# TravisWheelerLab/BATH

Measured on AMD Instinct MI355X. Metric: DP Gcells/s + residues/s through bathsearch pipeline at 1/2/4/8 MI355X, higher is better.
Workload: dtype u8/i16 integer scores (SSV: exact binary16), f32 Forward

## Files before the change

bath_amd/csrc/bath_viterbi.hip:

```cpp
#include <algorithm>
#include <cstdlib>
#include <functional>

#include "bath_common.hpp"
#include "bath_kernels.hpp"
#include "bath_launch.hpp"

using namespace bath;

namespace bath {

__device__ __forceinline__ s16x2 pk_adds(s16x2 a, s16x2 b) { return __builtin_elementwise_add_sat(a, b); }
__device__ __forceinline__ s16x2 pk_max(s16x2 a, s16x2 b) { return __builtin_elementwise_max(a, b); }
__device__ __forceinline__ s16x2 as_s2(unsigned v) { return __builtin_bit_cast(s16x2, v); }
__device__ __forceinline__ unsigned as_u(s16x2 v) { return __builtin_bit_cast(unsigned, v); }

struct VitLaneTables {
  const int16_t *rw;
  int rw_pitch_bytes;
  const uint32_t *tw2;
  const int16_t *rank;
};

struct VitLaneConsts {
  int M, base_w, xwE_loop, xwE_move, Q8;
  float scale_w;
  double invP_vit, invP_msv;
  float scale_b;
  int base_b, tec_b, bias_b;
};

typedef uint32_t u32x16 __attribute__((ext_vector_type(16)));

template <int NR>
#ifndef BATH_VIT_WAVES
#define BATH_VIT_WAVES 1
#endif
__global__ __launch_bounds__(256, (NR <= 76 ? BATH_VIT_WAVES : 1)) void vit_lane_kernel(SeqView sq, VitLaneTables tb, const uint32_t *__restrict__ tw2g, VitLaneConsts c, const int16_t *__restrict__ xwmove_tab,
                                                          const uint8_t *__restrict__ tjb_tab, const int32_t *__restrict__ todo, int64_t ntodo,
                                                          const int *__restrict__ ntodo_dev, const int *__restrict__ skip_dev, float *__restrict__ sc, int32_t *__restrict__ status,
                                                          const float *__restrict__ filtersc, const uint8_t *__restrict__ ssv_scores,
                                                          WindowRec *__restrict__ wins, int *__restrict__ win_count, int win_cap, int32_t *__restrict__ kminmax) {
  extern __shared__ __attribute__((aligned(16))) char lds[];
  char *s_rw = lds;
  int16_t *s_rank = reinterpret_cast<int16_t *>(lds + 30 * tb.rw_pitch_bytes);
  {
    const uint32_t *src = reinterpret_cast<const uint32_t *>(tb.rw);
    uint32_t *dst = reinterpret_cast<uint32_t *>(s_rw);
    for (int i = threadIdx.x; i < 30 * tb.rw_pitch_bytes / 4; i += blockDim.x) dst[i] = src[i];
    for (int i = threadIdx.x; i < 2 * NR; i += blockDim.x) s_rank[i] = tb.rank[i];
  }
  __syncthreads();
  if (ntodo_dev) ntodo = *ntodo_dev;
  const int64_t t = (int64_t)blockIdx.x * blockDim.x + threadIdx.x + (skip_dev ? *skip_dev : 0);
  if (t - (threadIdx.x & 63) >= ntodo) return;
  const bool live = t < ntodo;
  const int64_t sid = live ? (todo ? (int64_t)todo[t] : t) : (todo ? (int64_t)todo[0] : 0);
  const int L = live ? sq.len[sid] : 0;
  const uint8_t *s = sq.data + sq.off[sid];
  const int Lw = wave_max_i32(L);
  const bool do_win = (wins != nullptr);
  const int M = c.M;

  const int xw_move = xwmove_tab[L];
  int sc_thresh = 0, sc_ext_thresh = 0, skip_until = 0, kmin = 1 << 30, kmax = 0;
  if (do_win && live) {
    const double fsc = (double)filtersc[sid];
    sc_thresh = (int)(int16_t)(int)ceil(((fsc + 0.69314718055994529 * c.invP_vit + 3.0) * (double)c.scale_w) -
                                        (double)(float)c.xwE_move - (double)(float)xw_move + (double)(float)c.base_w);
    sc_ext_thresh = (int)ceil(((fsc + 0.69314718055994529 * c.invP_msv + 3.0) * (double)c.scale_b) + c.base_b + c.tec_b + (int)tjb_tab[L]);
  }
  const s16x2 NEG = {-32768, -32768};
  s16x2 Mr[NR], Ir[NR], Dr[NR];
#pragma unroll
  for (int r = 0; r < NR; r++) Mr[r] = Ir[r] = Dr[r] = NEG;
  int xN = c.base_w;
  int xB = (int16_t)(xN + xw_move);
  int xJ = -32768, xC = -32768;
  bool overflow = false;
  short ePrev = -32768;

  uint32_t wnext = (0 < L) ? *reinterpret_cast<const uint32_t *>(s) : 0x1d1d1d1du;
  for (int i0 = 0; i0 < Lw; i0 += 4) {
    const uint32_t w = wnext;
    wnext = (i0 + 4 < L) ? *reinterpret_cast<const uint32_t *>(s + i0 + 4) : 0x1d1d1d1du;
#pragma unroll 1
    for (int j = 0; j < 4; j++) {
      const int i = i0 + j + 1;
      const bool on = (i <= L) && !overflow;
      int x = (w >> (8 * j)) & 0xff;
      x = (i <= L) ? min(x, kKp - 1) : 29;
      const char *rowbase = s_rw + x * tb.rw_pitch_bytes;
      const s16x2 xBv = {(short)xB, (short)xB};
      s16x2 xEv = NEG;
      unsigned pM = (as_u(Mr[NR - 1]) << 16) | 0x8000u, pI = (as_u(Ir[NR - 1]) << 16) | 0x8000u, pD = (as_u(Dr[NR - 1]) << 16) | 0x8000u;
      s16x2 dpk = NEG;
      s16x2 cpk = {(short)-32768, ePrev};
      int twz = 0;
      asm volatile("" : "+s"(twz));
      const uint32_t *tw = tw2g + twz;
      u32x16 t_c, t_n;
      int4 e_c = *reinterpret_cast<const int4 *>(rowbase), e_n = e_c;
      asm volatile("s_load_dwordx16 %0, %1, 0x0" : "=s"(t_c) : "s"(tw));
#pragma unroll
      for (int r = 0; r < NR; r += 2) {
        asm volatile("s_waitcnt lgkmcnt(0)" ::: "memory");
        __builtin_amdgcn_sched_barrier(0);
        if ((r & 3) == 0 && r + 4 < NR) e_n = *reinterpret_cast<const int4 *>(rowbase + 4 * (r + 4));
        if (r + 2 < NR) asm volatile("s_load_dwordx16 %0, %1, %2" : "=s"(t_n) : "s"(tw), "i"((r + 2) * 32));
        __builtin_amdgcn_sched_barrier(0);
        const unsigned em[2] = {(r & 3) ? (unsigned)e_c.z : (unsigned)e_c.x, (r & 3) ? (unsigned)e_c.w : (unsigned)e_c.y};
#pragma unroll
        for (int q = 0; q < 2; q++) {
          const int rr = r + q;
          const unsigned tMM = t_c[8 * q + 0], tIM = t_c[8 * q + 1], tDM = t_c[8 * q + 2], tBM = t_c[8 * q + 3];
          const unsigned tMD = t_c[8 * q + 4], tDD = t_c[8 * q + 5], tMI = t_c[8 * q + 6], tII = t_c[8 * q + 7];
          const unsigned oM = as_u(Mr[rr]), oI = as_u(Ir[rr]);
          const unsigned oD = as_u(pk_max(Dr[rr], cpk));
          cpk = pk_adds(cpk, as_s2(tDD));
          const s16x2 ms = as_s2(pM), is = as_s2(pI), ds = as_s2(pD);
          s16x2 sv = pk_adds(xBv, as_s2(tBM));
          sv = pk_max(sv, pk_adds(ms, as_s2(tMM)));
          sv = pk_max(sv, pk_adds(is, as_s2(tIM)));
          sv = pk_max(sv, pk_adds(ds, as_s2(tDM)));
          sv = pk_adds(sv, as_s2(em[q]));
          Ir[rr] = pk_max(pk_adds(as_s2(oM), as_s2(tMI)), pk_adds(as_s2(oI), as_s2(tII)));
          const s16x2 dcv = pk_adds(sv, as_s2(tMD));
          xEv = pk_max(xEv, sv);
          Mr[rr] = sv;
          Dr[rr] = dpk;
          dpk = pk_max(dcv, pk_adds(dpk, as_s2(tDD)));
          pM = oM; pI = oI; pD = oD;
        }
        if (r + 2 < NR) t_c = t_n;
        if ((r & 3) == 2 && r + 2 < NR) e_c = e_n;
        asm volatile("" : "+v"(Mr[r]), "+v"(Mr[r + 1]), "+v"(Ir[r]), "+v"(Ir[r + 1]), "+v"(Dr[r]), "+v"(Dr[r + 1]), "+v"(dpk), "+v"(cpk), "+v"(xEv));
        __builtin_amdgcn_sched_barrier(0);
      }
      ePrev = dpk.x;
      if (on) {
        const int xE = max((int)xEv.x, (int)xEv.y);
        if (xE >= 32767) overflow = true;
        else {
          xN = (int16_t)(xN + 0);
          xC = (int16_t)max(xC + 0, xE + c.xwE_move);
          xJ = (int16_t)max(xJ + 0, xE + c.xwE_loop);
          xB = (int16_t)max(xJ + xw_move, xN + xw_move);
          if (do_win && i > skip_until && xE >= sc_thresh) {
            int rank = 32767;
#pragma unroll
            for (int r = 0; r < NR; r++) {
              if ((int)Mr[r].x == xE) rank = min(rank, (int)s_rank[2 * r]);
              if ((int)Mr[r].y == xE) rank = min(rank, (int)s_rank[2 * r + 1]);
            }
            const int k_start = (rank / 8) + c.Q8 * (rank % 8) + 1;
            int max_k_end = k_start, max_i_end = i, sc_ext = sc_ext_thresh, max_sc_ext = sc_ext, since = 0;
            int kk = k_start + 1, nn = i + 1;
            while (kk <= M && nn <= L) {
              sc_ext += c.bias_b - (int)ssv_scores[(size_t)kk * kKp + min((int)s[nn - 1], kKp - 1)];
              if (sc_ext >= max_sc_ext) { max_sc_ext = sc_ext; max_k_end = kk; max_i_end = nn; since = 0; }
              else if (++since == 5) break;
              kk++; nn++;
            }
            const int slot = atomicAdd(win_count, 1);
            if (slot < win_cap) wins[slot] = WindowRec{(int32_t)sid, i, max_k_end, max_k_end - k_start + 1, 0.0f};
            kmax = max(kmax, max_k_end);
            kmin = min(kmin, k_start);
            skip_until = max_i_end;
          }
        }
      }
    }
  }
  if (live) {
    if (overflow) { sc[sid] = INFINITY; status[sid] = BATH_ERANGE; }
    else if (xC > -32768) {
      float r = (float)xC + (float)xw_move - (float)c.base_w;
      r /= c.scale_w;
      r = (float)((double)r - 3.0);
      sc[sid] = r; status[sid] = BATH_OK;
    } else { sc[sid] = -INFINITY; status[sid] = BATH_OK; }
    if (do_win && kminmax) { kminmax[2 * sid] = kmin; kminmax[2 * sid + 1] = kmax; }
  }
}

constexpr int kLenBins = 2048;
constexpr int kVitLongTarget = 128;
__device__ __forceinline__ void len_block_range(int n, int &lo, int &hi) {
  const int per = (n + (int)gridDim.x - 1) / (int)gridDim.x;
  lo = min(n, (int)blockIdx.x * per); hi = min(n, lo + per);
}
__global__ __launch_bounds__(256) void len_hist_kernel(const int32_t *__restrict__ todo, const int *__restrict__ ntodo_dev, const int32_t *__restrict__ len,
                                                       int *__restrict__ hist) {
  __shared__ int s_cnt[kLenBins];
  for (int i = threadIdx.x; i < kLenBins; i += blockDim.x) s_cnt[i] = 0;
  __syncthreads();
  int lo, hi;
  len_block_range(*ntodo_dev, lo, hi);
  for (int j = lo + threadIdx.x; j < hi; j += blockDim.x) atomicAdd(&s_cnt[min(len[todo[j]], kLenBins - 1)], 1);
  __syncthreads();
  for (int i = threadIdx.x; i < kLenBins; i += blockDim.x) if (s_cnt[i]) atomicAdd(&hist[i], s_cnt[i]);
}
__global__ void len_scan_kernel(int *__restrict__ hist ) {
  __shared__ int tmp[kLenBins];
  for (int i = threadIdx.x; i < kLenBins; i += blockDim.x) tmp[i] = hist[i];
  __syncthreads();
  if (threadIdx.x == 0) {
    int run = 0;
    for (int b = kLenBins - 1; b >= 0; b--) { const int cnt = tmp[b]; tmp[b] = run; run += cnt; }
  }
  __syncthreads();
  for (int i = threadIdx.x; i < kLenBins; i += blockDim.x) hist[i] = tmp[i];
}
__global__ __launch_bounds__(256) void len_scatter_kernel(const int32_t *__restrict__ todo, const int *__restrict__ ntodo_dev, const int32_t *__restrict__ len,
                                                          int *__restrict__ cursor, int32_t *__restrict__ sorted) {
  __shared__ int s_cnt[kLenBins];
  for (int i = threadIdx.x; i < kLenBins; i += blockDim.x) s_cnt[i] = 0;
  __syncthreads();
  int lo, hi;
  len_block_range(*ntodo_dev, lo, hi);
  for (int j = lo + threadIdx.x; j < hi; j += blockDim.x) atomicAdd(&s_cnt[min(len[todo[j]], kLenBins - 1)], 1);
  __syncthreads();
  for (int i = threadIdx.x; i < kLenBins; i += blockDim.x) { const int c = s_cnt[i]; if (c) s_cnt[i] = atomicAdd(&cursor[i], c); }
  __syncthreads();
  for (int j = lo + threadIdx.x; j < hi; j += blockDim.x) {
    const int cnd = todo[j];
    sorted[atomicAdd(&s_cnt[min(len[cnd], kLenBins - 1)], 1)] = cnd;
  }
}

int vit_lane_supported(const bath_hip_oprofile *om) { return om->vit_NR > 0; }

const int *len_sort_count_longer(const int *d_bins, int T) { return d_bins + std::min(T + 1, kLenBins - 1); }

int launch_len_sort(bath_hip_ctx *ctx, const int32_t *d_todo, const int *d_ntodo, const int32_t *d_len, int *d_bins, int32_t *d_sorted) {
  BATH_HIP_TRY(ctx, hipMemsetAsync(d_bins, 0, kLenBins * sizeof(int), ctx->stream));
  hipLaunchKernelGGL(len_hist_kernel, dim3(256), dim3(256), 0, ctx->stream, d_todo, d_ntodo, d_len, d_bins);
  hipLaunchKernelGGL(len_scan_kernel, dim3(1), dim3(256), 0, ctx->stream, d_bins);
  hipLaunchKernelGGL(len_scatter_kernel, dim3(256), dim3(256), 0, ctx->stream, d_todo, d_ntodo, d_len, d_bins, d_sorted);
  BATH_HIP_TRY(ctx, hipGetLastError());
  return BATH_OK;
}

int launch_vit_lane(bath_hip_ctx *ctx, const bath_hip_oprofile *om, SeqView v, const int32_t *d_todo, int64_t ntodo, const int *ntodo_dev,
                    float *d_sc, int32_t *d_status, const VitWindowArgs *wa, const int *skip_dev) {
  if (ntodo == 0) return BATH_OK;
  VitLaneTables tb{om->d_vit_rw, om->vit_rw_pitch, om->d_vit_tw2, om->d_vit_rank};
  VitLaneConsts c{};
  c.M = om->M; c.base_w = om->base_w; c.xwE_loop = om->xw_E[0]; c.xwE_move = om->xw_E[1]; c.Q8 = std::max(2, ((om->M - 1) / 8) + 1);
  c.scale_w = om->scale_w; c.scale_b = om->scale_b; c.base_b = om->base_b; c.tec_b = om->tec_b; c.bias_b = om->bias_b;
  const float *fsc = nullptr; const uint8_t *ssv = nullptr; WindowRec *wins = nullptr; int *wc = nullptr; int cap = 0; int32_t *kmm = nullptr;
  if (wa) { c.invP_vit = wa->invP_vit; c.invP_msv = wa->invP_msv; fsc = wa->d_filtersc; ssv = wa->d_ssv_scores; wins = (WindowRec *)wa->d_wins; wc = wa->d_win_count; cap = wa->win_cap; kmm = wa->d_kminmax; }
  const int NRv = om->vit_NR;
  const size_t shmem = (size_t)30 * om->vit_rw_pitch + (size_t)2 * NRv * 2 + 16;
  const int blocks = (int)((ntodo + 255) / 256);
  bool launched = false;
#define BATH_VITL_CASE(N)                                                                                                              \
  if (!launched && NRv == N) {                                                                                                         \
    hipLaunchKernelGGL(vit_lane_kernel<N>, dim3(blocks), dim3(256), shmem, ctx->stream, v, tb, tb.tw2, c, om->lt.d_xwmove, om->lt.d_tjb, d_todo, ntodo, \
                       ntodo_dev, skip_dev, d_sc, d_status, fsc, ssv, wins, wc, cap, kmm);                                                       \
    launched = true;                                                                                                                   \
  }
  BATH_VITL_CASE(16) BATH_VITL_CASE(32) BATH_VITL_CASE(48) BATH_VITL_CASE(64) BATH_VITL_CASE(68) BATH_VITL_CASE(72) BATH_VITL_CASE(76) BATH_VITL_CASE(80)
  BATH_VITL_CASE(96) BATH_VITL_CASE(112)
#undef BATH_VITL_CASE
  if (!launched) { ctx->set_error("lane-per-target Viterbi kernel: unsupported model length"); return BATH_EINVAL; }
  BATH_HIP_TRY(ctx, hipGetLastError());
  return BATH_OK;
}

int64_t lane_min_nt() {
  static const int64_t v = [] { const char *e = std::getenv("BATH_HIP_LANE_MIN_NT"); return e ? std::atoll(e) : (int64_t)150'000'000; }();
  return v;
}

const char *vit_lane_kernel_name(const bath_hip_oprofile *om) {
#define BATH_VITL_NAME(N) if (om->vit_NR == N) return "vit_lane_kernel<" #N ">";
  BATH_VITL_NAME(16) BATH_VITL_NAME(32) BATH_VITL_NAME(48) BATH_VITL_NAME(64) BATH_VITL_NAME(68) BATH_VITL_NAME(72) BATH_VITL_NAME(76) BATH_VITL_NAME(80)
  BATH_VITL_NAME(96) BATH_VITL_NAME(112)
#undef BATH_VITL_NAME
  return "vit_lane_kernel<?>";
}

int launch_vit_sorted(bath_hip_ctx *ctx, const bath_hip_oprofile *om, SeqView v, const int32_t *d_todo, int64_t cap, const int *d_ntodo, const int32_t *d_len,
                      int *d_bins, int32_t *d_sorted, float *d_sc, int32_t *d_status, const VitWindowArgs *wa, const std::function<int(hipStream_t)> &beside) {
  int st;
  if ((st = launch_len_sort(ctx, d_todo, d_ntodo, d_len, d_bins, d_sorted)) != BATH_OK) return st;
  if (!ctx->side_stream) {
    BATH_HIP_TRY(ctx, hipStreamCreateWithFlags(&ctx->side_stream, hipStreamNonBlocking));
    BATH_HIP_TRY(ctx, hipEventCreateWithFlags(&ctx->ev_fork, hipEventDisableTiming));
    BATH_HIP_TRY(ctx, hipEventCreateWithFlags(&ctx->ev_join, hipEventDisableTiming));
  }
  static const int long_orf = [] { const char *e = std::getenv("BATH_HIP_VIT_LONG"); return e ? std::atoi(e) : kVitLongTarget; }();
  const int *d_nlong = len_sort_count_longer(d_bins, long_orf);
  BATH_HIP_TRY(ctx, hipEventRecord(ctx->ev_fork, ctx->stream));
  BATH_HIP_TRY(ctx, hipStreamWaitEvent(ctx->side_stream, ctx->ev_fork, 0));
  {
    hipStream_t main_stream = ctx->stream;
    ctx->stream = ctx->side_stream;
    st = launch_vit_wave(ctx, om, v, d_sorted, cap, d_sc, d_status, wa, d_nlong);
    ctx->stream = main_stream;
    if (st != BATH_OK) return st;
    if (beside && (st = beside(ctx->side_stream)) != BATH_OK) return st;
  }
  BATH_HIP_TRY(ctx, hipEventRecord(ctx->ev_join, ctx->side_stream));
  if ((st = launch_vit_lane(ctx, om, v, d_sorted, cap, d_ntodo, d_sc, d_status, wa, d_nlong)) != BATH_OK) return st;
  BATH_HIP_TRY(ctx, hipStreamWaitEvent(ctx->stream, ctx->ev_join, 0));
  return BATH_OK;
}

}
```

Baseline: 198.2 billion.

## Spill per-lane Viterbi scalars to LDS frame and software-pipeline the M recurrence

Result: no change. 199.8 billion (median of 6 runs) (+0.8%).

```diff
diff --git a/bath_amd/csrc/bath_viterbi.hip b/bath_amd/csrc/bath_viterbi.hip
--- a/bath_amd/csrc/bath_viterbi.hip
+++ b/bath_amd/csrc/bath_viterbi.hip
@@ -31,12 +31,14 @@
 };
 
 typedef uint32_t u32x16 __attribute__((ext_vector_type(16)));
+typedef uint32_t u32x4 __attribute__((ext_vector_type(4)));
+
+enum { VF_W, VF_L, VF_SLO, VF_SHI, VF_SID, VF_XB, VF_XJ, VF_XC, VF_EPREV, VF_XWMOVE, VF_OVF, VF_THRESH, VF_SKIP, VF_KMIN, VF_KMAX, kVitFrameSlots };
+constexpr int vit_lane_waves(int NR) { return NR <= 76 ? 2 : 1; }
+static size_t vit_lane_frame_off(int rw_pitch_bytes, int NR) { return ((size_t)30 * rw_pitch_bytes + (size_t)4 * NR + 15) & ~(size_t)15; }
 
 template <int NR>
-#ifndef BATH_VIT_WAVES
-#define BATH_VIT_WAVES 1
-#endif
-__global__ __launch_bounds__(256, (NR <= 76 ? BATH_VIT_WAVES : 1)) void vit_lane_kernel(SeqView sq, VitLaneTables tb, const uint32_t *__restrict__ tw2g, VitLaneConsts c, const int16_t *__restrict__ xwmove_tab,
+__global__ __launch_bounds__(256, vit_lane_waves(NR)) void vit_lane_kernel(SeqView sq, VitLaneTables tb, const uint32_t *__restrict__ tw2g, VitLaneConsts c, const int16_t *__restrict__ xwmove_tab,
                                                           const uint8_t *__restrict__ tjb_tab, const int32_t *__restrict__ todo, int64_t ntodo,
                                                           const int *__restrict__ ntodo_dev, const int *__restrict__ skip_dev, float *__restrict__ sc, int32_t *__restrict__ status,
                                                           const float *__restrict__ filtersc, const uint8_t *__restrict__ ssv_scores,
@@ -44,6 +46,8 @@
   extern __shared__ __attribute__((aligned(16))) char lds[];
   char *s_rw = lds;
   int16_t *s_rank = reinterpret_cast<int16_t *>(lds + 30 * tb.rw_pitch_bytes);
+  int *fr = reinterpret_cast<int *>(lds + ((30 * tb.rw_pitch_bytes + 4 * NR + 15) & ~15)) + threadIdx.x;
+#define FR(k) ((k) * 256)
   {
     const uint32_t *src = reinterpret_cast<const uint32_t *>(tb.rw);
     uint32_t *dst = reinterpret_cast<uint32_t *>(s_rw);
@@ -52,111 +56,146 @@
   }
   __syncthreads();
   if (ntodo_dev) ntodo = *ntodo_dev;
-  const int64_t t = (int64_t)blockIdx.x * blockDim.x + threadIdx.x + (skip_dev ? *skip_dev : 0);
-  if (t - (threadIdx.x & 63) >= ntodo) return;
-  const bool live = t < ntodo;
-  const int64_t sid = live ? (todo ? (int64_t)todo[t] : t) : (todo ? (int64_t)todo[0] : 0);
-  const int L = live ? sq.len[sid] : 0;
-  const uint8_t *s = sq.data + sq.off[sid];
-  const int Lw = wave_max_i32(L);
   const bool do_win = (wins != nullptr);
-  const int M = c.M;
-
-  const int xw_move = xwmove_tab[L];
-  int sc_thresh = 0, sc_ext_thresh = 0, skip_until = 0, kmin = 1 << 30, kmax = 0;
-  if (do_win && live) {
-    const double fsc = (double)filtersc[sid];
-    sc_thresh = (int)(int16_t)(int)ceil(((fsc + 0.69314718055994529 * c.invP_vit + 3.0) * (double)c.scale_w) -
-                                        (double)(float)c.xwE_move - (double)(float)xw_move + (double)(float)c.base_w);
-    sc_ext_thresh = (int)ceil(((fsc + 0.69314718055994529 * c.invP_msv + 3.0) * (double)c.scale_b) + c.base_b + c.tec_b + (int)tjb_tab[L]);
+  int Lw;
+  uint32_t wnext;
+  {
+    const int64_t t = (int64_t)blockIdx.x * blockDim.x + threadIdx.x + (skip_dev ? *skip_dev : 0);
+    if (t - (threadIdx.x & 63) >= ntodo) return;
+    const bool live = t < ntodo;
+    const int64_t sid = live ? (todo ? (int64_t)todo[t] : t) : (todo ? (int64_t)todo[0] : 0);
+    const int L = live ? sq.len[sid] : 0;
+    const uint8_t *s = sq.data + sq.off[sid];
+    Lw = wave_max_i32(L);
+    const int xw_move = xwmove_tab[L];
+    int sc_thresh = 0;
+    if (do_win && live) {
+      const double fsc = (double)filtersc[sid];
+      sc_thresh = (int)(int16_t)(int)ceil(((fsc + 0.69314718055994529 * c.invP_vit + 3.0) * (double)c.scale_w) -
+                                          (double)(float)c.xwE_move - (double)(float)xw_move + (double)(float)c.base_w);
+    }
+    wnext = (0 < L) ? *reinterpret_cast<const uint32_t *>(s) : 0x1d1d1d1du;
+    fr[FR(VF_L)] = L; fr[FR(VF_SLO)] = (int)(uint32_t)(uintptr_t)s; fr[FR(VF_SHI)] = (int)(uint32_t)((uintptr_t)s >> 32);
+    fr[FR(VF_SID)] = (int)sid;
+    fr[FR(VF_XB)] = (int16_t)(c.base_w + xw_move); fr[FR(VF_XJ)] = -32768; fr[FR(VF_XC)] = -32768;
+    fr[FR(VF_EPREV)] = -32768;
+    fr[FR(VF_XWMOVE)] = xw_move; fr[FR(VF_OVF)] = 0;
+    fr[FR(VF_THRESH)] = sc_thresh; fr[FR(VF_SKIP)] = 0; fr[FR(VF_KMIN)] = 1 << 30; fr[FR(VF_KMAX)] = 0;
   }
   const s16x2 NEG = {-32768, -32768};
   s16x2 Mr[NR], Ir[NR], Dr[NR];
 #pragma unroll
   for (int r = 0; r < NR; r++) Mr[r] = Ir[r] = Dr[r] = NEG;
-  int xN = c.base_w;
-  int xB = (int16_t)(xN + xw_move);
-  int xJ = -32768, xC = -32768;
-  bool overflow = false;
-  short ePrev = -32768;
-
-  uint32_t wnext = (0 < L) ? *reinterpret_cast<const uint32_t *>(s) : 0x1d1d1d1du;
+
   for (int i0 = 0; i0 < Lw; i0 += 4) {
-    const uint32_t w = wnext;
-    wnext = (i0 + 4 < L) ? *reinterpret_cast<const uint32_t *>(s + i0 + 4) : 0x1d1d1d1du;
+    {
+      fr[FR(VF_W)] = (int)wnext;
+      const uint8_t *s = reinterpret_cast<const uint8_t *>((uintptr_t)(uint32_t)fr[FR(VF_SLO)] | ((uintptr_t)(uint32_t)fr[FR(VF_SHI)] << 32));
+      wnext = (i0 + 4 < fr[FR(VF_L)]) ? *reinterpret_cast<const uint32_t *>(s + i0 + 4) : 0x1d1d1d1du;
+    }
 #pragma unroll 1
     for (int j = 0; j < 4; j++) {
       const int i = i0 + j + 1;
-      const bool on = (i <= L) && !overflow;
-      int x = (w >> (8 * j)) & 0xff;
-      x = (i <= L) ? min(x, kKp - 1) : 29;
-      const char *rowbase = s_rw + x * tb.rw_pitch_bytes;
-      const s16x2 xBv = {(short)xB, (short)xB};
+      const char *rowbase;
+      s16x2 xBv, cpk;
+      {
+        int x = ((uint32_t)fr[FR(VF_W)] >> (8 * j)) & 0xff;
+        x = (i <= fr[FR(VF_L)]) ? min(x, kKp - 1) : 29;
+        rowbase = s_rw + x * tb.rw_pitch_bytes;
+        const short xB = (short)fr[FR(VF_XB)];
+        xBv = s16x2{xB, xB};
+        cpk = s16x2{(short)-32768, (short)fr[FR(VF_EPREV)]};
+      }
       s16x2 xEv = NEG;
-      unsigned pM = (as_u(Mr[NR - 1]) << 16) | 0x8000u, pI = (as_u(Ir[NR - 1]) << 16) | 0x8000u, pD = (as_u(Dr[NR - 1]) << 16) | 0x8000u;
-      s16x2 dpk = NEG;
-      s16x2 cpk = {(short)-32768, ePrev};
       int twz = 0;
       asm volatile("" : "+s"(twz));
       const uint32_t *tw = tw2g + twz;
       u32x16 t_c, t_n;
-      int4 e_c = *reinterpret_cast<const int4 *>(rowbase), e_n = e_c;
-      asm volatile("s_load_dwordx16 %0, %1, 0x0" : "=s"(t_c) : "s"(tw));
+      u32x4 t_0;
+      int2 e_c = *reinterpret_cast<const int2 *>(rowbase), e_n = e_c;
+      asm volatile("s_load_dwordx4 %0, %1, 0x0" : "=s"(t_0) : "s"(tw));
+      asm volatile("s_load_dwordx16 %0, %1, %2" : "=s"(t_c) : "s"(tw), "i"(NR > 2 ? 12 : 0));
+      asm volatile("s_waitcnt lgkmcnt(0)" ::: "memory");
+      s16x2 nxt = pk_adds(as_s2((as_u(Mr[NR - 1]) << 16) | 0x8000u), as_s2(t_0[0]));
+      nxt = pk_max(nxt, pk_adds(as_s2((as_u(Ir[NR - 1]) << 16) | 0x8000u), as_s2(t_0[1])));
+      nxt = pk_max(nxt, pk_adds(as_s2((as_u(Dr[NR - 1]) << 16) | 0x8000u), as_s2(t_0[2])));
+      s16x2 oD = pk_max(Dr[0], cpk);
+      Dr[0] = NEG;
+      s16x2 dlast = NEG;
 #pragma unroll
       for (int r = 0; r < NR; r += 2) {
-        asm volatile("s_waitcnt lgkmcnt(0)" ::: "memory");
+        constexpr int kLastSh = NR > 2 ? 3 : 0;
+        const int sh = (r + 2 < NR) ? 0 : kLastSh;
+        if (r) asm volatile("s_waitcnt lgkmcnt(0)" ::: "memory");
         __builtin_amdgcn_sched_barrier(0);
-        if ((r & 3) == 0 && r + 4 < NR) e_n = *reinterpret_cast<const int4 *>(rowbase + 4 * (r + 4));
-        if (r + 2 < NR) asm volatile("s_load_dwordx16 %0, %1, %2" : "=s"(t_n) : "s"(tw), "i"((r + 2) * 32));
+        if (r + 2 < NR) e_n = *reinterpret_cast<const int2 *>(rowbase + 4 * (r + 2));
+        if (r + 4 < NR) asm volatile("s_load_dwordx16 %0, %1, %2" : "=s"(t_n) : "s"(tw), "i"((r + 2) * 32 + 12));
+        else if (r + 2 < NR) asm volatile("s_load_dwordx16 %0, %1, %2" : "=s"(t_n) : "s"(tw), "i"((r + 2) * 32));
         __builtin_amdgcn_sched_barrier(0);
-        const unsigned em[2] = {(r & 3) ? (unsigned)e_c.z : (unsigned)e_c.x, (r & 3) ? (unsigned)e_c.w : (unsigned)e_c.y};
+        const unsigned em[2] = {(unsigned)e_c.x, (unsigned)e_c.y};
 #pragma unroll
         for (int q = 0; q < 2; q++) {
           const int rr = r + q;
-          const unsigned tMM = t_c[8 * q + 0], tIM = t_c[8 * q + 1], tDM = t_c[8 * q + 2], tBM = t_c[8 * q + 3];
-          const unsigned tMD = t_c[8 * q + 4], tDD = t_c[8 * q + 5], tMI = t_c[8 * q + 6], tII = t_c[8 * q + 7];
-          const unsigned oM = as_u(Mr[rr]), oI = as_u(Ir[rr]);
-          const unsigned oD = as_u(pk_max(Dr[rr], cpk));
-          cpk = pk_adds(cpk, as_s2(tDD));
-          const s16x2 ms = as_s2(pM), is = as_s2(pI), ds = as_s2(pD);
-          s16x2 sv = pk_adds(xBv, as_s2(tBM));
-          sv = pk_max(sv, pk_adds(ms, as_s2(tMM)));
-          sv = pk_max(sv, pk_adds(is, as_s2(tIM)));
-          sv = pk_max(sv, pk_adds(ds, as_s2(tDM)));
+          const unsigned tBM = t_c[8 * q + sh + 0], tMD = t_c[8 * q + sh + 1], tDD = t_c[8 * q + sh + 2], tMI = t_c[8 * q + sh + 3], tII = t_c[8 * q + sh + 4];
+          const s16x2 oM = Mr[rr], oI = Ir[rr];
+          s16x2 sv = pk_max(pk_adds(xBv, as_s2(tBM)), nxt);
+          const s16x2 aMI = pk_adds(oM, as_s2(tMI)), aII = pk_adds(oI, as_s2(tII));
+          if (rr + 1 < NR) {
+            const unsigned tMMn = t_c[8 * q + sh + 5], tIMn = t_c[8 * q + sh + 6], tDMn = t_c[8 * q + sh + 7];
+            const s16x2 aMM = pk_adds(oM, as_s2(tMMn)), aIM = pk_adds(oI, as_s2(tIMn));
+            nxt = pk_max(pk_max(aMM, aIM), pk_adds(oD, as_s2(tDMn)));
+            asm volatile("" : "+v"(sv) : "v"(aMM), "v"(aIM));
+          }
+          asm volatile("" : "+v"(sv) : "v"(aMI), "v"(aII));
           sv = pk_adds(sv, as_s2(em[q]));
-          Ir[rr] = pk_max(pk_adds(as_s2(oM), as_s2(tMI)), pk_adds(as_s2(oI), as_s2(tII)));
-          const s16x2 dcv = pk_adds(sv, as_s2(tMD));
+          Ir[rr] = pk_max(aMI, aII);
+          Mr[rr] = sv;
           xEv = pk_max(xEv, sv);
-          Mr[rr] = sv;
-          Dr[rr] = dpk;
-          dpk = pk_max(dcv, pk_adds(dpk, as_s2(tDD)));
-          pM = oM; pI = oI; pD = oD;
+          s16x2 dcv = pk_adds(sv, as_s2(tMD));
+          if (rr + 1 < NR) {
+            cpk = pk_adds(cpk, as_s2(tDD));
+            oD = pk_max(Dr[rr + 1], cpk);
+            asm volatile("" : "+v"(dcv) : "v"(oD));
+            Dr[rr + 1] = pk_max(dcv, pk_adds(Dr[rr], as_s2(tDD)));
+          } else dlast = pk_max(dcv, pk_adds(Dr[rr], as_s2(tDD)));
         }
-        if (r + 2 < NR) t_c = t_n;
-        if ((r & 3) == 2 && r + 2 < NR) e_c = e_n;
-        asm volatile("" : "+v"(Mr[r]), "+v"(Mr[r + 1]), "+v"(Ir[r]), "+v"(Ir[r + 1]), "+v"(Dr[r]), "+v"(Dr[r + 1]), "+v"(dpk), "+v"(cpk), "+v"(xEv));
+        if (r + 2 < NR) { t_c = t_n; e_c = e_n; }
+        if (r + 2 < NR) asm volatile("" : "+v"(Mr[r]), "+v"(Mr[r + 1]), "+v"(Ir[r]), "+v"(Ir[r + 1]), "+v"(Dr[r + 1]), "+v"(Dr[r + 2]), "+v"(nxt), "+v"(oD), "+v"(cpk), "+v"(xEv));
+        else asm volatile("" : "+v"(Mr[r]), "+v"(Mr[r + 1]), "+v"(Ir[r]), "+v"(Ir[r + 1]), "+v"(Dr[r + 1]), "+v"(dlast), "+v"(xEv));
         __builtin_amdgcn_sched_barrier(0);
       }
-      ePrev = dpk.x;
-      if (on) {
+      asm volatile("" ::: "memory");
+      fr[FR(VF_EPREV)] = dlast.x;
+      const int L = fr[FR(VF_L)];
+      if ((i <= L) && !fr[FR(VF_OVF)]) {
         const int xE = max((int)xEv.x, (int)xEv.y);
-        if (xE >= 32767) overflow = true;
+        if (xE >= 32767) fr[FR(VF_OVF)] = 1;
         else {
-          xN = (int16_t)(xN + 0);
-          xC = (int16_t)max(xC + 0, xE + c.xwE_move);
-          xJ = (int16_t)max(xJ + 0, xE + c.xwE_loop);
-          xB = (int16_t)max(xJ + xw_move, xN + xw_move);
-          if (do_win && i > skip_until && xE >= sc_thresh) {
+          const int xw_move = fr[FR(VF_XWMOVE)];
+          const int xN = c.base_w;
+          const int xC = (int16_t)max(fr[FR(VF_XC)] + 0, xE + c.xwE_move);
+          const int xJ = (int16_t)max(fr[FR(VF_XJ)] + 0, xE + c.xwE_loop);
+          fr[FR(VF_XC)] = xC; fr[FR(VF_XJ)] = xJ;
+          fr[FR(VF_XB)] = (int16_t)max(xJ + xw_move, xN + xw_move);
+          if (do_win && i > fr[FR(VF_SKIP)] && xE >= fr[FR(VF_THRESH)]) {
             int rank = 32767;
 #pragma unroll
             for (int r = 0; r < NR; r++) {
               if ((int)Mr[r].x == xE) rank = min(rank, (int)s_rank[2 * r]);
               if ((int)Mr[r].y == xE) rank = min(rank, (int)s_rank[2 * r + 1]);
             }
+            const int sid = fr[FR(VF_SID)];
+            const uint8_t *s = reinterpret_cast<const uint8_t *>((uintptr_t)(uint32_t)fr[FR(VF_SLO)] | ((uintptr_t)(uint32_t)fr[FR(VF_SHI)] << 32));
+            uint32_t ip_lo = (uint32_t)__builtin_bit_cast(uint64_t, c.invP_msv), ip_hi = (uint32_t)(__builtin_bit_cast(uint64_t, c.invP_msv) >> 32);
+            float scale_b = c.scale_b;
+            int add_b = c.base_b + c.tec_b;
+            asm volatile("" : "+s"(ip_lo), "+s"(ip_hi), "+s"(scale_b), "+s"(add_b));
+            const double invP_msv = __builtin_bit_cast(double, ((uint64_t)ip_hi << 32) | ip_lo);
+            const int sc_ext_thresh = (int)ceil((((double)filtersc[sid] + 0.69314718055994529 * invP_msv + 3.0) * (double)scale_b) + add_b + (int)tjb_tab[L]);
             const int k_start = (rank / 8) + c.Q8 * (rank % 8) + 1;
             int max_k_end = k_start, max_i_end = i, sc_ext = sc_ext_thresh, max_sc_ext = sc_ext, since = 0;
             int kk = k_start + 1, nn = i + 1;
-            while (kk <= M && nn <= L) {
+            while (kk <= c.M && nn <= L) {
               sc_ext += c.bias_b - (int)ssv_scores[(size_t)kk * kKp + min((int)s[nn - 1], kKp - 1)];
               if (sc_ext >= max_sc_ext) { max_sc_ext = sc_ext; max_k_end = kk; max_i_end = nn; since = 0; }
               else if (++since == 5) break;
@@ -164,24 +203,31 @@
             }
             const int slot = atomicAdd(win_count, 1);
             if (slot < win_cap) wins[slot] = WindowRec{(int32_t)sid, i, max_k_end, max_k_end - k_start + 1, 0.0f};
-            kmax = max(kmax, max_k_end);
-            kmin = min(kmin, k_start);
-            skip_until = max_i_end;
+            fr[FR(VF_KMAX)] = max(fr[FR(VF_KMAX)], max_k_end);
+            fr[FR(VF_KMIN)] = min(fr[FR(VF_KMIN)], k_start);
+            fr[FR(VF_SKIP)] = max_i_end;
           }
         }
       }
+      asm volatile("" ::: "memory");
     }
   }
-  if (live) {
-    if (overflow) { sc[sid] = INFINITY; status[sid] = BATH_ERANGE; }
+  int tid = threadIdx.x;
+  asm volatile("" : "+v"(tid));
+  const int64_t t = (int64_t)blockIdx.x * blockDim.x + tid + (skip_dev ? *skip_dev : 0);
+  if (t < ntodo) {
+    const int64_t sid = todo ? (int64_t)fr[FR(VF_SID)] : t;
+    const int xC = fr[FR(VF_XC)];
+    if (fr[FR(VF_OVF)]) { sc[sid] = INFINITY; status[sid] = BATH_ERANGE; }
     else if (xC > -32768) {
-      float r = (float)xC + (float)xw_move - (float)c.base_w;
+      float r = (float)xC + (float)fr[FR(VF_XWMOVE)] - (float)c.base_w;
       r /= c.scale_w;
       r = (float)((double)r - 3.0);
       sc[sid] = r; status[sid] = BATH_OK;
     } else { sc[sid] = -INFINITY; status[sid] = BATH_OK; }
-    if (do_win && kminmax) { kminmax[2 * sid] = kmin; kminmax[2 * sid + 1] = kmax; }
-  }
+    if (do_win && kminmax) { kminmax[2 * sid] = fr[FR(VF_KMIN)]; kminmax[2 * sid + 1] = fr[FR(VF_KMAX)]; }
+  }
+#undef FR
 }
 
 constexpr int kLenBins = 2048;
@@ -252,7 +298,7 @@
   const float *fsc = nullptr; const uint8_t *ssv = nullptr; WindowRec *wins = nullptr; int *wc = nullptr; int cap = 0; int32_t *kmm = nullptr;
   if (wa) { c.invP_vit = wa->invP_vit; c.invP_msv = wa->invP_msv; fsc = wa->d_filtersc; ssv = wa->d_ssv_scores; wins = (WindowRec *)wa->d_wins; wc = wa->d_win_count; cap = wa->win_cap; kmm = wa->d_kminmax; }
   const int NRv = om->vit_NR;
-  const size_t shmem = (size_t)30 * om->vit_rw_pitch + (size_t)2 * NRv * 2 + 16;
+  const size_t shmem = vit_lane_frame_off(om->vit_rw_pitch, NRv) + (size_t)kVitFrameSlots * 256 * sizeof(int);
   const int blocks = (int)((ntodo + 255) / 256);
   bool launched = false;
 #define BATH_VITL_CASE(N)                                                                                                              \
```
